# fernandezdaniel/MOBOCMF

Hardware: AMD Instinct MI355X
Metric: ELBO steps/sec (MFDGP d=8 M=512 N=8192 S=8) (higher is better)
Workload: dtype f64

## Files before the change

mobocmf_amd/csrc/common.h:

```cpp
#pragma once
#include <hip/hip_runtime.h>
#include <stdint.h>

#include "../../include/mobocmf_hip.h"

#define TILE 128
#define NB 64

static inline int64_t round_up(int64_t v, int64_t m) { return (v + m - 1) / m * m; }

#define HIP_TRY(expr)                                   \
    do {                                                \
        hipError_t _e = (expr);                         \
        if (_e != hipSuccess) return MOBOCMF_HIP_ERROR; \
    } while (0)

const mobocmf_tuning& tune();
bool tuning_ok(const mobocmf_tuning* t);
void probe_at(int i, hipStream_t s);
struct TuneScope {
    const mobocmf_tuning* prev_t;
    void* const* prev_p;
    explicit TuneScope(const mobocmf_tuning* t, void* const* probe = nullptr);
    ~TuneScope();
    TuneScope(const TuneScope&) = delete;
    TuneScope& operator=(const TuneScope&) = delete;
};

enum { TRI_NONE = 0, TRI_LOWER_A = 1, TRI_UPPER_A = 2, TRI_LOWER_B = 4, TRI_UPPER_B = 8 };
enum { EPI_STORE = 0, EPI_COLSTATS = 1, EPI_DA = 2 };

struct GemmArgs {
    const double* A;
    const double* B;
    double* C;
    int64_t lda, ldb, ldc;
    int Mr;
    int64_t Nc;
    int64_t Kd;
    int tri;
    int lower_out;
    int sym_out;
    int sym_full;
    int splitk_diag;
    double alpha;
    int accumulate;
    int rm;
    int pair_mode;
    int64_t slab_stride;
    int64_t strideA, strideB, strideC;
    int batched;
    int zlayers;
    int64_t zsA, zsB, zsC;
    const double* bscale;
    int64_t Kreal;
    double* rowdot_part;
    int stream_out;
    const int32_t* skip_if_zero;
    const int32_t* dual_flag;
    const double* bscale2;
    double* C2;
    const int32_t* colact;
    const int32_t* kact;
    int epi;
    double* colsq_part;
    double* coldot_part;
    const double* avec;
    const double* gmu;
    const double* cgv;
    const double* Aaux;
};

int launch_gemm(const GemmArgs& g, bool B_T, int splitk, hipStream_t s);
int gemm_nt_slabs(const GemmArgs& g, int splitk);
bool gemm_nt_is_small(const GemmArgs& g);
int gemm_rowdot_parts(const GemmArgs& g);
int gemm_colstat_rows(const GemmArgs& g);
int launch_gemm_auto(const GemmArgs& g, bool B_T, double* ws, int64_t ws_elems, hipStream_t s);
int launch_gemm_auto_pair(const GemmArgs& a, const GemmArgs& b, double* ws, int64_t ws_elems, hipStream_t s);

#define MAX_ZL 4

struct GramArgs {
    int kind, d, xdiv, zdiv;
    const double* x;
    const double* f;
    int64_t nbase;
    const double* Zx;
    const double* zf;
    int M;
    const double* hyp;
    double* K;
    int64_t ldk;
    int Mp;
    int64_t Np;
    double* knn;
    double jitter;
    int is_kmm;
    int gm;
    const double* G;
    const double* gknn;
    double* hyp_part;
    double* df_part;
    double* dzf_part;
    double* dx_part;
    const int32_t* colact;
};
int launch_gram_fwd(const GramArgs& g, hipStream_t s);
int launch_gram_bwd(const GramArgs& g, bool want_dx, hipStream_t s);
void gram_grid(const GramArgs& g, dim3* grid);
struct SumTask {
    const double* part; int64_t P, stride;
    const double* part2; int64_t P2, stride2;
    double* out; int64_t len; int accumulate;
    const double* extra;
};
int launch_sum_partials_multi(const SumTask* tasks, int n, hipStream_t s);

int launch_trtri(const double* L, int64_t ld, int Mp, const double* Dinv, double* Linv, double* T, double* ws,
                 int64_t ws_elems, hipStream_t s);
int launch_potrf_z(double* A, int64_t ld, int Mp, int M, double* Dinv, double* Ld, int32_t* const* info, int nz, int64_t zs,
                   double* zero0, double* zero1, void* sync, int* inverse_done, hipStream_t s);
int launch_trtri_z(const double* L, int64_t ld, int Mp, const double* Dinv, double* Linv, double* T, double* ws,
                   int64_t ws_elems, int nz, int64_t zs, hipStream_t s);

int launch_zero32(void* ptr, int64_t nwords, hipStream_t s);
int launch_pad_vec(const double* src, int64_t n, double* dst, int64_t np, hipStream_t s);
int launch_gemv_rows(const double* Mat, int64_t ld, const double* vec, double* out, int rows, int64_t cols, double scale,
                     int accumulate, hipStream_t s);
int launch_moments_finish(const double* qpart, const double* mupart, const double* rpart, int nrb, int64_t Np, int64_t N,
                          const double* knn, int branch, double min_var, double* q, double* r, double* varraw,
                          double* mean, double* var, int32_t* zero_word, hipStream_t s);
int launch_moments_bwd_prep(const double* g_mean, const double* g_var, const double* knn, const double* q,
                            const double* varraw, int branch, double min_var, int64_t N, int64_t Np, double* gmu,
                            double* gv, double* gv2, double* cgv, int32_t* nclamped, int zeroed, int32_t* blkact, hipStream_t s);
int launch_reduce_slabs_sym(const double* slabs, int64_t slab_stride, int nslab, int nslab_diag, double* out, int Mp, const int32_t* flag,
                            const double* fallback, hipStream_t s);
int launch_reduce_slabs_sym2(const double* slabs, const double* slabs2, int64_t slab_stride, int nslab, int nslab_diag,
                             double* out, double* out2, int Mp, const int32_t* flag, hipStream_t s);
int launch_copy_block(const double* src, int64_t lds, double* dst, int64_t ldd, int64_t rows, int64_t cols, hipStream_t s);
int launch_mf_combine(const double* Ks, const double* Kn, int64_t ld, const double* s1, const double* s2, const int32_t* l1,
                      const int32_t* l2, const double* ntab, int64_t n1, int64_t n2, double diag, double* out, int64_t ldo,
                      int64_t rows_p, int64_t cols_p, hipStream_t s);
int launch_copy_pad_identity(const double* src, int64_t lds, int n, double* dst, int np, hipStream_t s);
int launch_exact_gp_mll(const double* L, int64_t ld, const double* a, int n, double* mll, hipStream_t s);
int launch_exact_gp_finish(const double* qpart, const double* mupart, int nparts, int64_t ntp, int64_t nt, const double* kss,
                           double* mean, double* var, hipStream_t s);
int launch_mirror_lower(const double* src, int64_t lds, double* dst, int64_t ldd, int64_t row0, int64_t rows, int64_t cols,
                        int64_t n_real, hipStream_t s);
int launch_chain_outputs_z(const double* X, const double* LSp, const double* LinvT, const double* da_tot, int M, int Mp,
                           const double* const* gkl, double* const* gLS, double* const* gm, int nz, int64_t zs, hipStream_t s);
int launch_transpose_z(const double* in, int64_t ldi, double* out, int64_t ldo, int64_t rows, int64_t cols, int nz,
                       int64_t zs, hipStream_t s);
int launch_gemv_rows_z(const double* Mat, int64_t ld, const double* vec, double* out, int rows, int64_t cols, double scale,
                       int accumulate, int nz, int64_t zs, hipStream_t s);
int launch_transpose_pad_z(const double* in, double* out, int Mp, const double* const* LS, const double* const* m, int M,
                           double* LSp, double* mp, int nz, int64_t zs, hipStream_t s);
int launch_transpose_gemv_z(const double* in, double* out, int Mp, const double* Mat, const double* vec, double* vout, int nz,
                            int64_t zs, hipStream_t s);
int launch_kl_z(const double* L, const double* LSp, const double* U, const double* a, int M, int Mp, double* const* kl,
                double* part, int nz, int64_t zs, hipStream_t s);
int launch_dutot_y_z(const double* G1, const double* G2, const double* Hc, const double* U, const double* da, const double* a,
                     const double* const* gkl, int Mp, double* dU, double* da_tot, double* Y, int nz, int64_t zs, hipStream_t s);
int launch_dl_from_t2_z(const double* T2, const double* L, const double* const* gkl, int M, int Mp, double* dL, int nz,
                        int64_t zs, hipStream_t s);
int launch_phi_z(const double* T3, int Mp, double* P, int nz, int64_t zs, hipStream_t s);
int launch_symmetrize_z(const double* S, int Mp, double* G, int nz, int64_t zs, hipStream_t s);

enum { FCS_L = 0, FCS_LINV = 1, FCS_LINVT = 2, FCS_U = 3, FCS_UT = 4, FCS_LS = 5, FCS_A = 6 };
int launch_frozen_predict(const mobocmf_frozen_predict_model* host_models, const mobocmf_frozen_predict_model* dev_models,
                          int n_models, bool input_gradients, hipStream_t s);
int launch_frozen_predict_split(const mobocmf_frozen_predict_model* host_models, const mobocmf_frozen_predict_model* dev_models,
                                int n_models, bool input_gradients, hipStream_t s);

static inline int hyp_len(int kind, int d) { return kind == 0 ? 1 + d : 5 + 2 * d; }
#define MAX_D MOBOCMF_MAX_D

#define PHILOX_M0 0xD2511F53u
#define PHILOX_M1 0xCD9E8D57u
#define PHILOX_W0 0x9E3779B9u
#define PHILOX_W1 0xBB67AE85u
__device__ __forceinline__ void philox4x32_10(uint32_t c0, uint32_t c1, uint32_t c2, uint32_t c3, uint32_t k0, uint32_t k1,
                                              uint32_t (&out)[4]) {
#pragma unroll
    for (int r = 0; r < 10; ++r) {
        const uint32_t hi0 = __umulhi(PHILOX_M0, c0), lo0 = PHILOX_M0 * c0;
        const uint32_t hi1 = __umulhi(PHILOX_M1, c2), lo1 = PHILOX_M1 * c2;
        c0 = hi1 ^ c1 ^ k0; c1 = lo1; c2 = hi0 ^ c3 ^ k1; c3 = lo0;
        k0 += PHILOX_W0; k1 += PHILOX_W1;
    }
    out[0] = c0; out[1] = c1; out[2] = c2; out[3] = c3;
}
__device__ __forceinline__ double philox_normal(uint64_t seed, uint64_t call, uint64_t idx) {
    uint32_t r[4];
    philox4x32_10((uint32_t)idx, (uint32_t)(idx >> 32), (uint32_t)call, (uint32_t)(call >> 32), (uint32_t)seed,
                  (uint32_t)(seed >> 32), r);
    const double u1 = ((double)(((uint64_t)(r[0] >> 5) << 26) | (uint64_t)(r[1] >> 6)) + 0.5) * 1.1102230246251565e-16;
    const double u2 = ((double)(((uint64_t)(r[2] >> 5) << 26) | (uint64_t)(r[3] >> 6)) + 0.5) * 1.1102230246251565e-16;
    return sqrt(-2.0 * log(u1)) * cospi(2.0 * u2);
}
__device__ __forceinline__ double philox_uniform(uint64_t seed, uint64_t call, uint64_t idx) {
    uint32_t r[4];
    philox4x32_10((uint32_t)idx, (uint32_t)(idx >> 32), (uint32_t)call, (uint32_t)(call >> 32), (uint32_t)seed,
                  (uint32_t)(seed >> 32), r);
    return ((double)(((uint64_t)(r[0] >> 5) << 26) | (uint64_t)(r[1] >> 6)) + 0.5) * 1.1102230246251565e-16;
}
```

mobocmf_amd/csrc/gemm_f64.hip:

```cpp
#include "common.h"
#include <type_traits>
#include <atomic>

typedef double v4f64 __attribute__((ext_vector_type(4)));
typedef double v2f64 __attribute__((ext_vector_type(2)));

#define BM 128
#define BN 128
#define BK 16
#define KL_MAX 1024
#define TILE_ELEMS (BM * BK)

#define IMG_SWZ(row) ((((row) >> 1) & 1) | ((((row) >> 3) & 1) << 2))


template <int CTRL>
__device__ __forceinline__ double dpp_mov(double v) {
    int lo = __double2loint(v), hi = __double2hiint(v);
    lo = __builtin_amdgcn_update_dpp(0, lo, CTRL, 0xF, 0xF, false);
    hi = __builtin_amdgcn_update_dpp(0, hi, CTRL, 0xF, 0xF, false);
    return __hiloint2double(hi, lo);
}
__device__ __forceinline__ double row16_sum(double v) {
    v += dpp_mov<0xB1>(v);
    v += dpp_mov<0x4E>(v);
    v += dpp_mov<0x141>(v);
    v += dpp_mov<0x140>(v);
    return v;
}
__device__ __forceinline__ double rows4_sum(double v) {
    {
        const unsigned lo = (unsigned)__double2loint(v), hi = (unsigned)__double2hiint(v);
        const auto rl = __builtin_amdgcn_permlane16_swap(lo, lo, false, false);
        const auto rh = __builtin_amdgcn_permlane16_swap(hi, hi, false, false);
        v = __hiloint2double((int)rh[0], (int)rl[0]) + __hiloint2double((int)rh[1], (int)rl[1]);
    }
    {
        const unsigned lo = (unsigned)__double2loint(v), hi = (unsigned)__double2hiint(v);
        const auto rl = __builtin_amdgcn_permlane32_swap(lo, lo, false, false);
        const auto rh = __builtin_amdgcn_permlane32_swap(hi, hi, false, false);
        v = __hiloint2double((int)rh[0], (int)rl[0]) + __hiloint2double((int)rh[1], (int)rl[1]);
    }
    return v;
}

__device__ __forceinline__ void glds16(const double* gsrc, double* lds_wave_base) {
    __builtin_amdgcn_global_load_lds((const __attribute__((address_space(1))) void*)gsrc,
                                     (__attribute__((address_space(3))) void*)lds_wave_base, 16, 0, 0);
}

#ifdef GEMM_STAMPS
__device__ unsigned long long* g_stamp_buf = nullptr;
extern "C" int mobocmf_debug_set_stamps(unsigned long long* p) {
    return hipMemcpyToSymbol(HIP_SYMBOL(g_stamp_buf), &p, sizeof(p)) == hipSuccess ? 0 : 3;
}
#define STAMP(i)                                                                                            \
    do {                                                                                                    \
        if (g_stamp_buf && threadIdx.x == 0) g_stamp_buf[(int64_t)blockIdx.x * 32 + (i)] = __builtin_amdgcn_s_memrealtime(); \
    } while (0)
#define STAMP_ID()                                                                                          \
    do {                                                                                                    \
        if (g_stamp_buf && threadIdx.x == 0) {                                                              \
            unsigned hw, xcc;                                                                               \
            asm volatile("s_getreg_b32 %0, hwreg(HW_REG_HW_ID)" : "=s"(hw));                               \
            asm volatile("s_getreg_b32 %0, hwreg(HW_REG_XCC_ID)" : "=s"(xcc));                             \
            g_stamp_buf[(int64_t)blockIdx.x * 32 + 15] = ((unsigned long long)xcc << 32) | hw;              \
        }                                                                                                   \
    } while (0)
#define STEP_STAMPS_DECL unsigned long long sst[10] = {0, 0, 0, 0, 0, 0, 0, 0, 0, 0};
#define STEP_STAMP(i) do { if (sbase >= 0) sst[sbase + (i)] = __builtin_amdgcn_s_memrealtime(); } while (0)
#define STEP_STAMPS_FLUSH                                                                                   \
    do {                                                                                                    \
        if (g_stamp_buf && threadIdx.x == 0)                                                                \
            for (int q = 0; q < 10; ++q) g_stamp_buf[(int64_t)blockIdx.x * 32 + 16 + q] = sst[q];           \
    } while (0)
#else
#define STAMP(i)
#define STAMP_ID()
#define STEP_STAMPS_DECL
#define STEP_STAMP(i)
#define STEP_STAMPS_FLUSH
#endif

template <bool B_T, bool TRI, int EPI, int RM>
__global__ __launch_bounds__(256, RM == 64 ? 3 : 2) void gemm_f64_kernel(GemmArgs g, int nrb, int64_t ncb, int splitk, int pair) {
    static_assert(RM == 128 || (RM == 64 && !B_T), "tile heights: 128, or 64 for the A B form");
    constexpr int MT = RM / 32;
    constexpr int A_ELEMS = RM * BK;
    constexpr int STAGE_ELEMS = A_ELEMS + TILE_ELEMS;
    __shared__ __attribute__((aligned(16))) double lds[2 * STAGE_ELEMS];
    __shared__ int kl[B_T ? KL_MAX : 1];
    __shared__ int kl_wsum[4];
    if (g.skip_if_zero && *g.skip_if_zero == 0) return;
    STAMP(0);
    STAMP_ID();
    int64_t id = blockIdx.x;
    if (g.dual_flag) {
        const int64_t half = (int64_t)(gridDim.x >> 1);
        if (id >= half) {
            if (*g.dual_flag == 0) return;
            id -= half;
            g.bscale = g.bscale2;
            g.C = g.C2;
        }
    }
    int rb, z = 0, sk_eff = splitk;
    int64_t cb;
    if (g.batched) {
        z = blockIdx.z;
        cb = id / nrb;
        rb = nrb - 1 - (int)(id % nrb);
    } else if (splitk > 1 && g.lower_out && g.splitk_diag > 0) {
        const int64_t nF = (int64_t)nrb * (nrb - 1) / 2, nblkF = nF * splitk;
        const bool diag = id >= nblkF;
        const int64_t id2 = diag ? id - nblkF : id, nT = diag ? nrb : nF;
        sk_eff = diag ? g.splitk_diag : splitk;
        int64_t t;
        if ((sk_eff & 7) == 0 && (nblkF & 7) == 0) {
            const int64_t xcd = id2 & 7, seq = id2 >> 3;
            t = seq % nT;
            z = (int)((seq / nT) * 8 + xcd);
        } else {
            t = id2 % nT;
            z = (int)(id2 / nT);
        }
        if (diag) {
            rb = (int)t;
            cb = t;
        } else {
            int r = 1;
            while ((int64_t)r * (r + 1) / 2 <= t) ++r;
            rb = r;
            cb = t - (int64_t)r * (r - 1) / 2;
        }
    } else if (splitk > 1) {
        const int64_t ntile = g.lower_out ? (int64_t)nrb * (nrb + 1) / 2 : (int64_t)nrb * ncb;
        int64_t t;
        if ((splitk & 7) == 0) {
            const int64_t xcd = id & 7, seq = id >> 3;
            t = seq % ntile;
            z = (int)((seq / ntile) * 8 + xcd);
        } else {
            t = id % ntile;
            z = (int)(id / ntile);
        }
        if (g.lower_out) {
            int r = 0;
            while ((int64_t)(r + 1) * (r + 2) / 2 <= t) ++r;
            rb = r;
            cb = t - (int64_t)r * (r + 1) / 2;
        } else {
            cb = t / nrb;
            rb = (int)(t % nrb);
        }
    } else {
        const int nslot = pair ? (nrb + 1) / 2 : nrb;
        int sl;
        if ((ncb & 7) == 0) {
            int64_t xcd = id & 7, slot = id >> 3;
            cb = (slot / nslot) * 8 + xcd;
            sl = (int)(slot % nslot);
        } else {
            cb = id / nslot;
            sl = (int)(id % nslot);
        }
        rb = pair ? sl : nrb - 1 - sl;
    }
    if (g.lower_out && cb > rb) return;

    const double* A = g.A;
    const double* B = g.B;
    double* C = g.C;
    if (g.batched) {
        const int zl = g.zlayers > 1 ? z % g.zlayers : 0;
        const int zb = g.zlayers > 1 ? z / g.zlayers : z;
        A += zb * g.strideA + zl * g.zsA;
        B += zb * g.strideB + zl * g.zsB;
        C += zb * g.strideC + zl * g.zsC;
    }
    if (!g.batched && splitk > 1) {
        C += z * g.slab_stride;
        if (g.zlayers > 1) {
            A += blockIdx.z * g.zsA;
            B += blockIdx.z * g.zsB;
            C += blockIdx.z * g.zsC;
        }
    }
    const int nparts = (pair && rb != nrb - 1 - rb) ? 2 : 1;
    const int rb_first = rb;

    const int tid = threadIdx.x;
    const int lane = tid & 63;
    const int wave = __builtin_amdgcn_readfirstlane(tid >> 6);
    const int wr = wave >> 1, wc = wave & 1;
    const int li = lane & 15, lk = lane >> 4;

    if constexpr (!B_T) {
        if (g.colact && g.colact[cb] == 0) {
            if (EPI == EPI_DA && g.rowdot_part) {
                for (int part = 0; part < nparts; ++part) {
                    const int rbp = part == 0 ? rb_first : nrb - 1 - rb_first;
                    for (int i = tid; i < 2 * RM; i += 256)
                        g.rowdot_part[((int64_t)cb * 2 + i / RM) * g.Mr + (int64_t)rbp * RM + i % RM] = 0.0;
                }
            }
            return;
        }
    }

    const int a_row = tid >> 3;
    const int a_lchk = (tid & 7) ^ IMG_SWZ(a_row);
    const double* Ag0 = A + (int64_t)a_row * g.lda + a_lchk * 2;
    const double* Bg = B_T ? B + (cb * BN + a_row) * g.ldb + a_lchk * 2
                           : B + (int64_t)wave * g.ldb + cb * BN;
    auto stage = [&](const double* Ag, int64_t k, int buf) {
        double* As = lds + buf * STAGE_ELEMS;
        double* Bs = As + A_ELEMS;
#pragma unroll
        for (int r = 0; r < RM / 32; ++r) glds16(Ag + (int64_t)(32 * r) * g.lda + k, As + (r * 4 + wave) * 128);
        if (B_T) {
#pragma unroll
            for (int r = 0; r < 4; ++r) glds16(Bg + (int64_t)(32 * r) * g.ldb + k, Bs + (r * 4 + wave) * 128);
        } else {
#pragma unroll
            for (int r = 0; r < 4; ++r)
                glds16(Bg + (k + 4 * r) * g.ldb + lane * 2, Bs + (r * 4 + wave) * 128);
        }
    };

    const int swA = IMG_SWZ(li);
    const int colP0 = ((2 * lk + 0) ^ swA) << 1, colP1 = ((2 * lk + 1) ^ swA) << 1;
    const int a_base = (wr * 16 + li) * BK;
    const int bt_base = (wc * 16 + li) * BK;
    const int bn_base = (4 * lk) * BN + wc * 64 + 2 * li;

  STEP_STAMPS_DECL
  for (int part = 0; part < nparts; ++part) {
    const bool upper = (g.tri & TRI_UPPER_A) != 0;
    const bool long_first_is_high = !upper;
    rb = ((part == 0) == long_first_is_high) ? nrb - 1 - rb_first : rb_first;
    if (nparts == 1) rb = rb_first;
    const bool rev = TRI && nparts == 2 && (upper ? part == 0 : part == 1);
    int64_t k0 = 0, k1 = g.Kd;
    if (g.tri & TRI_LOWER_A) {
        int64_t e = (int64_t)(rb + 1) * RM;
        if (k1 > e) k1 = e;
    }
    if (g.tri & TRI_UPPER_A) {
        int64_t b = (int64_t)rb * RM;
        if (k0 < b) k0 = b;
    }
    if (g.tri & TRI_LOWER_B) {
        int64_t b = cb * BN;
        if (k0 < b) k0 = b;
    }
    if (g.tri & TRI_UPPER_B) {
        int64_t e = (cb + 1) * BN;
        if (k1 > e) k1 = e;
    }
    bool compact = false;
    int64_t ct0 = 0;
    int co0 = 0;
    if (!g.batched && splitk > 1) {
        bool sliced = false;
        if constexpr (B_T) {
            if (g.kact) {
                const int nb = (int)(g.Kd / 128), run = (nb + 255) / 256;
                const int rb0 = tid * run < nb ? tid * run : nb, rb1 = rb0 + run < nb ? rb0 + run : nb;
                int cnt = 0;
                for (int b = rb0; b < rb1; ++b) cnt += g.kact[b] != 0 ? 1 : 0;
                int inc = cnt;
#pragma unroll
                for (int off = 1; off < 64; off <<= 1) {
                    const int v = __shfl_up(inc, off);
                    if (lane >= off) inc += v;
                }
                if (lane == 63) kl_wsum[wave] = inc;
                __syncthreads();
                int ord = inc - cnt;
                for (int w = 0; w < wave; ++w) ord += kl_wsum[w];
                const int64_t nkt = (int64_t)(kl_wsum[0] + kl_wsum[1] + kl_wsum[2] + kl_wsum[3]) * (128 / BK);
                const int64_t per = (nkt + sk_eff - 1) / sk_eff;
                const int64_t tb = z * per < nkt ? z * per : nkt, te = tb + per < nkt ? tb + per : nkt;
                ct0 = tb;
                co0 = (int)(tb / (128 / BK));
                const int co1 = te > tb ? (int)((te - 1) / (128 / BK)) : co0 - 1;
                for (int b = rb0; b < rb1; ++b)
                    if (g.kact[b] != 0) {
                        if (ord >= co0 && ord <= co1 && ord - co0 < KL_MAX) kl[ord - co0] = b;
                        ++ord;
                    }
                __syncthreads();
                compact = true;
                sliced = true;
                k0 = 0;
                k1 = (te - tb) * BK;
            }
        }
        if (!sliced) {
            int64_t nkt = k1 > k0 ? (k1 - k0) / BK : 0;
            int64_t per = (nkt + sk_eff - 1) / sk_eff;
            int64_t b = k0 + z * per * BK, e = b + per * BK;
            k0 = b < k1 ? b : k1;
            k1 = e < k1 ? e : k1;
        }
    }
    const double* Ag = Ag0 + (int64_t)rb * RM * g.lda;

    v4f64 acc[MT][4];
#pragma unroll
    for (int i = 0; i < MT; ++i)
#pragma unroll
        for (int j = 0; j < 4; ++j) acc[i][j] = (v4f64){0.0, 0.0, 0.0, 0.0};

    const int64_t nk = (k1 > k0) ? (k1 - k0) / BK : 0;
#define KSTEP(KT) (rev ? nk - 1 - (KT) : (KT))
    auto koff = [&](int64_t kt) -> int64_t {
        if (B_T && compact) {
            const int64_t t = ct0 + kt;
            return (int64_t)kl[(int)(t / (128 / BK)) - co0] * 128 + (t % (128 / BK)) * BK;
        }
        return k0 + KSTEP(kt) * BK;
    };
#define KOFF(KT) koff(KT)
    if (nk > 0) stage(Ag, KOFF(0), 0);

    asm volatile("s_waitcnt vmcnt(0)" ::: "memory");
    __syncthreads();
    STAMP(1 + 4 * part);
    v4f64 w_nxt = (v4f64){1.0, 1.0, 1.0, 1.0};
    if (B_T && g.bscale && nk > 0) w_nxt = *(const v4f64*)(g.bscale + KOFF(0) + 4 * lk);
    v2f64 fa[MT][2];
    double fb[4][4];
#define LOAD_A16(MT_)                                                                                       \
    fa[MT_][0] = *(const v2f64*)(As + a_base + (MT_) * 32 * BK + colP0);                                    \
    fa[MT_][1] = *(const v2f64*)(As + a_base + (MT_) * 32 * BK + colP1);
#define LOAD_B16                                                                                            \
    if (B_T) {                                                                                              \
        _Pragma("unroll") for (int t = 0; t < 4; ++t) {                                                    \
            const v2f64 v0 = *(const v2f64*)(Bs + bt_base + t * 32 * BK + colP0);                           \
            const v2f64 v1 = *(const v2f64*)(Bs + bt_base + t * 32 * BK + colP1);                           \
            fb[0][t] = v0[0];                                                                               \
            fb[1][t] = v0[1];                                                                               \
            fb[2][t] = v1[0];                                                                               \
            fb[3][t] = v1[1];                                                                               \
        }                                                                                                   \
        if (g.bscale) {                                                                                     \
// ... 1073 lines not shown
```

mobocmf_amd/csrc/gram.hip:

```cpp
#include "common.h"

#define GT 128
#define GM 32


typedef double v2f64_t __attribute__((ext_vector_type(2)));

template <int KIND, int DB, int XD>
__global__ __launch_bounds__(GT) void gram_fwd_kernel(GramArgs g) {
    __shared__ __attribute__((aligned(16))) double stg[XD ? (GT / 64) * 64 * (XD + 2) : 1];
    __shared__ double zs[GM][DB];
    __shared__ double zfs[GM];
    __shared__ double il1[DB], il2[DB];
    const int d = g.d;
    const int tid = threadIdx.x;
    const int gm = g.gm;
    const int m0 = blockIdx.y * gm;
    const double* hyp = g.hyp;
    double a1, af = 0, nu = 0, a2 = 0, ilf = 0;
    if (KIND == 0) {
        a1 = hyp[0];
        if (tid < DB) il1[tid] = tid < d ? 1.0 / hyp[1 + tid] : 0.0;
    } else {
        a1 = hyp[0]; af = hyp[1]; nu = hyp[2]; a2 = hyp[3]; ilf = 1.0 / hyp[4];
        if (tid < DB) { il1[tid] = tid < d ? 1.0 / hyp[5 + tid] : 0.0; il2[tid] = tid < d ? 1.0 / hyp[5 + d + tid] : 0.0; }
    }
    for (int e = tid; e < gm * DB; e += GT) {
        int mm = e / DB, k = e % DB;
        int m = m0 + mm;
        zs[mm][k] = (m < g.M && k < d) ? g.Zx[(int64_t)(m / g.zdiv) * d + k] : 0.0;
    }
    if (KIND == 1 && tid < gm) zfs[tid] = (m0 + tid < g.M) ? g.zf[m0 + tid] : 0.0;
    __syncthreads();

    const int64_t n0 = (int64_t)blockIdx.x * GT + tid;
    const int xdiv = XD ? XD : g.xdiv;
    const int64_t c0 = n0 * xdiv;
    if (c0 >= g.Np) return;
    const bool real = n0 < g.nbase;
    double xr[DB];
#pragma unroll
    for (int k = 0; k < DB; ++k) xr[k] = (real && k < d) ? g.x[n0 * d + k] : 0.0;
    double fr[XD ? XD : 1];
    if (XD && KIND == 1) {
#pragma unroll
        for (int s = 0; s < XD; s += 2) {
            v2f64_t v = real ? *(const v2f64_t*)(g.f + c0 + s) : (v2f64_t){0.0, 0.0};
            fr[s] = v[0];
            fr[s + 1] = v[1];
        }
    }

    const bool full_wave = XD && __ballot(real) == ~0ull;
    (void)full_wave;
    if (g.knn && blockIdx.y == 0) {
        for (int s = 0; s < xdiv; ++s) {
            int64_t n = c0 + s;
            if (n >= g.Np) break;
            double v = 0.0;
            if (real) {
                if (KIND == 0) v = a1;
                else { double fn = g.f[n]; v = a1 * (nu * fn * fn + af) + a2; }
            }
            g.knn[n] = v;
        }
    }
    for (int mm = 0; mm < gm; ++mm) {
        const int m = m0 + mm;
        double* krow = g.K + (int64_t)m * g.ldk;
        if (!real || m >= g.M) {
            for (int s = 0; s < xdiv; ++s) {
                int64_t n = c0 + s;
                if (n >= g.Np) break;
                krow[n] = (g.is_kmm && n == m) ? 1.0 : 0.0;
            }
            continue;
        }
        double d1 = 0.0, d2 = 0.0;
#pragma unroll
        for (int k = 0; k < DB; ++k) {
            double df = xr[k] - zs[mm][k];
            double t1 = df * il1[k];
            d1 += t1 * t1;
            if (KIND == 1) { double t2 = df * il2[k]; d2 += t2 * t2; }
        }
        const double E1 = exp(-0.5 * d1);
        if (KIND == 0) {
            double v = a1 * E1;
            if (g.is_kmm && c0 == m) v += g.jitter;
            krow[c0] = v;
            for (int s = 1; s < xdiv; ++s) krow[c0 + s] = a1 * E1;
        } else if (XD) {
            const double E2 = exp(-0.5 * d2);
            const double zfm = zfs[mm];
            const double c1 = a1 * E1, c2 = a2 * E2;
            const double cp = c1 * nu * zfm, cq = c1 * af;
            const int lane = tid & 63;
            double* my = stg + (tid >> 6) * 64 * (XD + 2);
#pragma unroll
            for (int s = 0; s < XD; s += 2) {
                v2f64_t v;
#pragma unroll
                for (int e = 0; e < 2; ++e) {
                    const double fn = fr[s + e];
                    const double fd = (fn - zfm) * ilf;
                    v[e] = cq * exp(-0.5 * fd * fd) + (cp * fn + c2);
                }
                if (full_wave) *(v2f64_t*)(my + lane * (XD + 2) + s) = v;
                else *(v2f64_t*)(krow + c0 + s) = v;
            }
            if (full_wave) {
                double* wrow = krow + (c0 - (int64_t)lane * XD);
#pragma unroll
                for (int i = 0; i < XD / 2; ++i) {
                    const int e = (i * 64 + lane) * 2;
                    *(v2f64_t*)(wrow + e) = *(const v2f64_t*)(my + (e / XD) * (XD + 2) + e % XD);
                }
            }
        } else {
            const double E2 = exp(-0.5 * d2);
            const double zfm = zfs[mm];
            const double c1 = a1 * E1, c2 = a2 * E2;
            for (int s = 0; s < xdiv; ++s) {
                const int64_t n = c0 + s;
                const double fn = g.f[n];
                const double fd = (fn - zfm) * ilf;
                const double Ef = exp(-0.5 * fd * fd);
                double v = c1 * (nu * fn * zfm + af * Ef) + c2;
                if (g.is_kmm && n == m) v += g.jitter;
                krow[n] = v;
            }
        }
    }
}

__device__ __forceinline__ double wave_sum(double v) {
    v += __shfl_xor(v, 1);
    v += __shfl_xor(v, 2);
    v += __shfl_xor(v, 4);
    v += __shfl_xor(v, 8);
    v += __shfl_xor(v, 16);
    v += __shfl_xor(v, 32);
    return v;
}

template <int KIND, int DB, bool WANT_DX, int XD>
__global__ __launch_bounds__(GT) void gram_bwd_kernel(GramArgs g) {
    __shared__ double zs[GM][DB];
    __shared__ double zfs[GM];
    __shared__ double il1[DB], il2[DB];
    __shared__ double dzf_s[GM];
    __shared__ double red[2][8 + 2 * DB];
    extern __shared__ double dfs[];
    const int d = g.d;
    const int tid = threadIdx.x, lane = tid & 63, wave = tid >> 6;
    const int gm = g.gm;
    const int m0 = blockIdx.y * gm;
    const double* hyp = g.hyp;
    double a1, af = 0, nu = 0, a2 = 0, ilf = 0;
    if (KIND == 0) {
        a1 = hyp[0];
        if (tid < DB) il1[tid] = tid < d ? 1.0 / hyp[1 + tid] : 0.0;
    } else {
        a1 = hyp[0]; af = hyp[1]; nu = hyp[2]; a2 = hyp[3]; ilf = 1.0 / hyp[4];
        if (tid < DB) { il1[tid] = tid < d ? 1.0 / hyp[5 + tid] : 0.0; il2[tid] = tid < d ? 1.0 / hyp[5 + d + tid] : 0.0; }
    }
    for (int e = tid; e < gm * DB; e += GT) {
        int mm = e / DB, k = e % DB;
        int m = m0 + mm;
        zs[mm][k] = (m < g.M && k < d) ? g.Zx[(int64_t)(m / g.zdiv) * d + k] : 0.0;
    }
    if (tid < gm) {
        dzf_s[tid] = 0.0;
        if (KIND == 1) zfs[tid] = (m0 + tid < g.M) ? g.zf[m0 + tid] : 0.0;
    }
    __syncthreads();

    const int64_t n0 = (int64_t)blockIdx.x * GT + tid;
    const int xdiv = XD ? XD : g.xdiv;
    const int64_t c0 = n0 * xdiv;
    const bool real = n0 < g.nbase;
    static_assert(XD == 0 || 128 % XD == 0, "replica runs must not straddle a column block");
    unsigned long long amask = ~0ull;
    if (g.colact && real) {
        if (XD) amask = g.colact[c0 >> 7] != 0 ? ~0ull : 0ull;
        else {
            amask = 0ull;
            for (int s = 0; s < xdiv; ++s) amask |= (unsigned long long)(g.colact[(c0 + s) >> 7] != 0 ? 1 : 0) << s;
        }
    }
    const bool live = real && amask != 0ull;
    double fr[XD ? XD : 1], dfa[XD ? XD : 1];
    if (XD) {
#pragma unroll
        for (int s = 0; s < XD; s += 2) {
            v2f64_t v = real ? *(const v2f64_t*)(g.f + c0 + s) : (v2f64_t){0.0, 0.0};
            fr[s] = v[0];
            fr[s + 1] = v[1];
            dfa[s] = dfa[s + 1] = 0.0;
        }
    }
    double xr[DB], aL1[DB], aL2[KIND == 1 ? DB : 1], aX[WANT_DX ? DB : 1];
#pragma unroll
    for (int k = 0; k < DB; ++k) {
        xr[k] = (real && k < d) ? g.x[n0 * d + k] : 0.0;
        aL1[k] = 0.0;
        if (KIND == 1) aL2[k] = 0.0;
        if (WANT_DX) aX[k] = 0.0;
    }
    double s_a1 = 0, s_af = 0, s_nu = 0, s_a2 = 0, s_lsf = 0;
    if (KIND == 1 && !XD)
        for (int s = 0; s < xdiv; ++s) dfs[s * GT + tid] = 0.0;

    if (g.gknn && blockIdx.y == 0 && real) {
        for (int s = 0; s < xdiv; ++s) {
            const int64_t n = c0 + s;
            const double gk = g.gknn[n];
            if (KIND == 0) s_a1 += gk;
            else {
                const double fn = g.f[n];
                s_a1 += gk * (nu * fn * fn + af);
                s_nu += gk * a1 * fn * fn;
                s_af += gk * a1;
                s_a2 += gk;
            }
        }
    }

    for (int mm = 0; mm < gm; ++mm) {
        const int m = m0 + mm;
        if (m >= g.M) break;
        double dzf_loc = 0.0;
        if (live) {
            const double* grow = g.G + (int64_t)m * g.ldk;
            double d1 = 0.0, d2 = 0.0;
#pragma unroll
            for (int k = 0; k < DB; ++k) {
                double df = xr[k] - zs[mm][k];
                double t1 = df * il1[k];
                d1 += t1 * t1;
                if (KIND == 1) { double t2 = df * il2[k]; d2 += t2 * t2; }
            }
            const double E1 = exp(-0.5 * d1);
            double W1 = 0.0, W2 = 0.0;
            if (KIND == 0) {
                double Gsum = 0.0;
                for (int s = 0; s < xdiv; ++s) Gsum += ((amask >> s) & 1ull) ? grow[c0 + s] : 0.0;
                s_a1 += Gsum * E1;
                W1 = Gsum * a1 * E1;
            } else {
                const double E2 = exp(-0.5 * d2);
                const double zfm = zfs[mm];
                const double aE1 = a1 * E1;
                const double c_a = aE1 * nu * zfm, c_b = aE1 * af * ilf;
                double G2s = 0.0, S1 = 0.0, S2 = 0.0, S3 = 0.0, S4 = 0.0;
                auto body = [&](double Gv, double fn, double& dfacc) {
                    const double fd = (fn - zfm) * ilf;
                    const double GEf = Gv * exp(-0.5 * fd * fd);
                    const double T = GEf * fd;
                    G2s += Gv;
                    S1 += Gv * fn;
                    S2 += GEf;
                    S3 += T;
                    S4 += T * fd;
                    dfacc += Gv * c_a - T * c_b;
                };
                if (XD) {
#pragma unroll
                    for (int s = 0; s < XD; s += 2) {
                        const v2f64_t Gp = *(const v2f64_t*)(grow + c0 + s);
                        body(Gp[0], fr[s], dfa[s]);
                        body(Gp[1], fr[s + 1], dfa[s + 1]);
                    }
                } else {
                    for (int s = 0; s < xdiv; ++s) {
                        double acc = 0.0;
                        body(((amask >> s) & 1ull) ? grow[c0 + s] : 0.0, g.f[c0 + s], acc);
                        dfs[s * GT + tid] += acc;
                    }
                }
                const double inner = nu * zfm * S1 + af * S2;
                s_a1 += E1 * inner;
                s_nu += aE1 * zfm * S1;
                s_af += aE1 * S2;
                s_lsf += c_b * S4;
                W1 = aE1 * inner;
                dzf_loc = aE1 * nu * S1 + c_b * S3;
                s_a2 += G2s * E2;
                W2 = G2s * a2 * E2;
            }
#pragma unroll
            for (int k = 0; k < DB; ++k) {
                double df = xr[k] - zs[mm][k];
                double t1 = df * il1[k];
                aL1[k] += W1 * t1 * t1;
                double gx = W1 * t1 * il1[k];
                if (KIND == 1) {
                    double t2 = df * il2[k];
                    aL2[k] += W2 * t2 * t2;
                    gx += W2 * t2 * il2[k];
                }
                if (WANT_DX) aX[k] -= gx;
            }
        }
        if (KIND == 1) {
            double tot = wave_sum(dzf_loc);
            if (lane == 0) atomicAdd(&dzf_s[mm], tot);
        }
    }
    if (KIND == 1) {
        for (int s = 0; s < xdiv; ++s) {
            const int64_t n = c0 + s;
            if (n >= g.Np) break;
            double v = real ? (XD ? dfa[XD ? s : 0] : dfs[s * GT + tid]) : 0.0;
            if (real && g.gknn && blockIdx.y == 0) v += g.gknn[n] * a1 * 2.0 * nu * g.f[n];
            g.df_part[(int64_t)blockIdx.y * g.Np + n] = v;
        }
    }
    if (WANT_DX && real) {
        double* dxp = g.dx_part + ((int64_t)blockIdx.y * g.nbase + n0) * d;
#pragma unroll
        for (int k = 0; k < DB; ++k)
            if (k < d) dxp[k] = aX[k];
    }
    const int H = (KIND == 0) ? 1 + d : 5 + 2 * d;
    {
        double v;
        v = wave_sum(s_a1); if (lane == 0) red[wave][0] = v;
        if (KIND == 1) {
            v = wave_sum(s_af); if (lane == 0) red[wave][1] = v;
            v = wave_sum(s_nu); if (lane == 0) red[wave][2] = v;
            v = wave_sum(s_a2); if (lane == 0) red[wave][3] = v;
            v = wave_sum(s_lsf); if (lane == 0) red[wave][4] = v;
        }
#pragma unroll
        for (int k = 0; k < DB; ++k) {
            if (k < d) {
                v = wave_sum(aL1[k]);
                if (lane == 0) red[wave][(KIND == 0 ? 1 : 5) + k] = v * il1[k];
                if (KIND == 1) {
                    v = wave_sum(aL2[k]);
                    if (lane == 0) red[wave][5 + d + k] = v * il2[k];
                }
            }
        }
    }
    __syncthreads();
    double* hp = g.hyp_part + ((int64_t)blockIdx.y * gridDim.x + blockIdx.x) * H;
    if (tid < H) hp[tid] = red[0][tid] + red[1][tid];
    if (KIND == 1 && tid < gm) g.dzf_part[(int64_t)blockIdx.x * g.Mp + m0 + tid] = dzf_s[tid];
}

#define SUM_MULTI_MAX 8
struct SumTasksArg { SumTask t[SUM_MULTI_MAX]; int blk0[SUM_MULTI_MAX + 1]; int wide[SUM_MULTI_MAX]; int n; };
__global__ void sum_partials_multi_kernel(SumTasksArg T) {
    __shared__ double sh[4];
    int k = 0;
    while (k + 1 < T.n && (int)blockIdx.x >= T.blk0[k + 1]) ++k;
    const SumTask& t = T.t[k];
    if (T.wide[k] == 1) {
        const int64_t j = (int64_t)(blockIdx.x - T.blk0[k]);
        double v = 0.0;
        for (int64_t p = threadIdx.x; p < t.P; p += 256) v += t.part[p * t.stride + j];
        if (t.part2)
            for (int64_t p = threadIdx.x; p < t.P2; p += 256) v += t.part2[p * t.stride2 + j];
        v += __shfl_xor(v, 1); v += __shfl_xor(v, 2); v += __shfl_xor(v, 4);
        v += __shfl_xor(v, 8); v += __shfl_xor(v, 16); v += __shfl_xor(v, 32);
        if ((threadIdx.x & 63) == 0) sh[threadIdx.x >> 6] = v;
        __syncthreads();
        if (threadIdx.x == 0) {
            v = sh[0] + sh[1] + sh[2] + sh[3];
            if (t.extra) v += t.extra[j];
            t.out[j] = t.accumulate ? t.out[j] + v : v;
        }
        return;
    }
    if (T.wide[k] == 2) {
        __shared__ double sq[4][64];
        const int jj = threadIdx.x & 63, q = threadIdx.x >> 6;
        const int64_t j = (int64_t)(blockIdx.x - T.blk0[k]) * 64 + jj;
        double v = 0.0;
        if (j < t.len) {
            for (int64_t p = q; p < t.P; p += 4) v += t.part[p * t.stride + j];
            if (t.part2)
                for (int64_t p = q; p < t.P2; p += 4) v += t.part2[p * t.stride2 + j];
        }
        sq[q][jj] = v;
        __syncthreads();
        if (q == 0 && j < t.len) {
            v = (sq[0][jj] + sq[1][jj]) + (sq[2][jj] + sq[3][jj]);
            if (t.extra) v += t.extra[j];
            t.out[j] = t.accumulate ? t.out[j] + v : v;
        }
        return;
    }
    const int64_t j = (int64_t)(blockIdx.x - T.blk0[k]) * blockDim.x + threadIdx.x;
    if (j >= t.len) return;
    double v = 0.0;
    for (int64_t p = 0; p < t.P; ++p) v += t.part[p * t.stride + j];
    if (t.part2)
        for (int64_t p = 0; p < t.P2; ++p) v += t.part2[p * t.stride2 + j];
    if (t.extra) v += t.extra[j];
    t.out[j] = t.accumulate ? t.out[j] + v : v;
}

int launch_sum_partials_multi(const SumTask* tasks, int n, hipStream_t s) {
    if (n > SUM_MULTI_MAX) {
        for (int i = 0; i < n; i += SUM_MULTI_MAX) {
            int rc = launch_sum_partials_multi(tasks + i, n - i < SUM_MULTI_MAX ? n - i : SUM_MULTI_MAX, s);
            if (rc) return rc;
        }
        return MOBOCMF_OK;
    }
    SumTasksArg T = {};
    int64_t nb = 0;
    int m = 0;
    for (int i = 0; i < n; ++i) {
        if (tasks[i].len <= 0) continue;
        T.t[m] = tasks[i];
        T.blk0[m] = (int)nb;
        const int64_t pmax = tasks[i].P > (tasks[i].part2 ? tasks[i].P2 : 0) ? tasks[i].P : tasks[i].P2;
        T.wide[m] = (pmax >= 64 && tasks[i].len <= 4096) ? 1 : (pmax >= 16 ? 2 : 0);
        nb += T.wide[m] == 1 ? tasks[i].len : T.wide[m] == 2 ? (tasks[i].len + 63) / 64 : (tasks[i].len + 255) / 256;
        ++m;
    }
    T.blk0[m] = (int)nb;
    T.n = m;
    if (m == 0) return MOBOCMF_OK;
    if (nb > 0x7fffffff) return MOBOCMF_BAD_ARG;
    hipLaunchKernelGGL(sum_partials_multi_kernel, dim3((unsigned)nb), dim3(256), 0, s, T);
    return hipGetLastError() == hipSuccess ? MOBOCMF_OK : MOBOCMF_HIP_ERROR;
}

static inline int d_bucket(int d) { return d <= 2 ? 2 : (d <= 8 ? 8 : 32); }

static int gram_rows_per_block(const GramArgs& g, bool fwd = false) {
    int64_t nb_cols = (g.Np + g.xdiv - 1) / g.xdiv;
    int64_t gx = (nb_cols + GT - 1) / GT;
    int gm = GM;
    while (gm > GM / 4 && gx * (g.Mp / gm) < 1024) gm /= 2;
    if (fwd && g.is_kmm)
        while (gm > 2 && gx * (g.Mp / gm) < 4096) gm /= 2;
    return gm;
}
void gram_grid(const GramArgs& g, dim3* grid) {
    int64_t nb_cols = (g.Np + g.xdiv - 1) / g.xdiv;
    *grid = dim3((unsigned)((nb_cols + GT - 1) / GT), (unsigned)(g.Mp / gram_rows_per_block(g)), 1);
}

int launch_gram_fwd(const GramArgs& g0, hipStream_t s) {
    GramArgs g = g0;
    g.gm = gram_rows_per_block(g0, true);
    if (g.d < 1 || g.d > 32) return MOBOCMF_BAD_ARG;
    dim3 grid;
    gram_grid(g, &grid);
    grid.y = (unsigned)(g.Mp / g.gm);
    const int db = d_bucket(g.d);
#define GF(K, D, X) hipLaunchKernelGGL((gram_fwd_kernel<K, D, X>), grid, dim3(GT), 0, s, g)
    const bool vec_ok = g.kind == 1 && !g.is_kmm && ((uintptr_t)g.f % 16 == 0) && ((uintptr_t)g.K % 16 == 0) && (g.ldk % 2 == 0);
    if (g.kind == 0) { if (db == 2) GF(0, 2, 0); else if (db == 8) GF(0, 8, 0); else GF(0, 32, 0); }
    else if (vec_ok && g.xdiv == 8) { if (db == 2) GF(1, 2, 8); else if (db == 8) GF(1, 8, 8); else GF(1, 32, 8); }
    else if (vec_ok && g.xdiv == 16) { if (db == 2) GF(1, 2, 16); else if (db == 8) GF(1, 8, 16); else GF(1, 32, 16); }
    else { if (db == 2) GF(1, 2, 0); else if (db == 8) GF(1, 8, 0); else GF(1, 32, 0); }
#undef GF
    return hipGetLastError() == hipSuccess ? MOBOCMF_OK : MOBOCMF_HIP_ERROR;
}

int launch_gram_bwd(const GramArgs& g0, bool want_dx, hipStream_t s) {
    GramArgs g = g0;
    g.gm = gram_rows_per_block(g0);
    if (g.d < 1 || g.d > 32) return MOBOCMF_BAD_ARG;
    dim3 grid;
    gram_grid(g, &grid);
    const int db = d_bucket(g.d);
    if (g.xdiv > 48) return MOBOCMF_BAD_ARG;
    const size_t shm = g.kind == 1 ? (size_t)g.xdiv * GT * sizeof(double) : 0;
#define GB(K, D, X)                                                                                    \
    do {                                                                                               \
        if (want_dx) hipLaunchKernelGGL((gram_bwd_kernel<K, D, true, X>), grid, dim3(GT), (X) ? 0 : shm, s, g);   \
        else hipLaunchKernelGGL((gram_bwd_kernel<K, D, false, X>), grid, dim3(GT), (X) ? 0 : shm, s, g);          \
    } while (0)
    const bool vec_ok = g.kind == 1 && ((uintptr_t)g.f % 16 == 0) && ((uintptr_t)g.G % 16 == 0) && (g.ldk % 2 == 0);
    if (g.kind == 0) { if (db == 2) GB(0, 2, 0); else if (db == 8) GB(0, 8, 0); else GB(0, 32, 0); }
    else if (vec_ok && g.xdiv == 8) { if (db == 2) GB(1, 2, 8); else if (db == 8) GB(1, 8, 8); else GB(1, 32, 8); }
    else if (vec_ok && g.xdiv == 16) { if (db == 2) GB(1, 2, 16); else if (db == 8) GB(1, 8, 16); else GB(1, 32, 16); }
    else { if (db == 2) GB(1, 2, 0); else if (db == 8) GB(1, 8, 0); else GB(1, 32, 0); }
#undef GB
    return hipGetLastError() == hipSuccess ? MOBOCMF_OK : MOBOCMF_HIP_ERROR;
}
```

Baseline: 1070.

## Restructure gram backward: stage G rows in LDS, prefetch, DPP reductions

Reworks the Gram backward kernel. It adds an XD==1 specialization that stages the block's G rows into shared memory up front. For XD>1 it software-prefetches the next G row into registers and keeps df accumulators in LDS instead of registers, and it vectorizes the x loads. Wave reductions now use DPP and permlane swaps instead of shfl_xor, and occupancy hints are added to launch_bounds. This targets load latency and register pressure in the backward pass, at the cost of more LDS use and template variants.

```diff
diff --git a/mobocmf_amd/csrc/common.h b/mobocmf_amd/csrc/common.h
--- a/mobocmf_amd/csrc/common.h
+++ b/mobocmf_amd/csrc/common.h
@@ -26,6 +26,37 @@
     TuneScope(const TuneScope&) = delete;
     TuneScope& operator=(const TuneScope&) = delete;
 };
+
+template <int CTRL>
+__device__ __forceinline__ double dpp_mov(double v) {
+    int lo = __double2loint(v), hi = __double2hiint(v);
+    lo = __builtin_amdgcn_update_dpp(0, lo, CTRL, 0xF, 0xF, false);
+    hi = __builtin_amdgcn_update_dpp(0, hi, CTRL, 0xF, 0xF, false);
+    return __hiloint2double(hi, lo);
+}
+__device__ __forceinline__ double row16_sum(double v) {
+    v += dpp_mov<0xB1>(v);
+    v += dpp_mov<0x4E>(v);
+    v += dpp_mov<0x141>(v);
+    v += dpp_mov<0x140>(v);
+    return v;
+}
+__device__ __forceinline__ double rows4_sum(double v) {
+    {
+        const unsigned lo = (unsigned)__double2loint(v), hi = (unsigned)__double2hiint(v);
+        const auto rl = __builtin_amdgcn_permlane16_swap(lo, lo, false, false);
+        const auto rh = __builtin_amdgcn_permlane16_swap(hi, hi, false, false);
+        v = __hiloint2double((int)rh[0], (int)rl[0]) + __hiloint2double((int)rh[1], (int)rl[1]);
+    }
+    {
+        const unsigned lo = (unsigned)__double2loint(v), hi = (unsigned)__double2hiint(v);
+        const auto rl = __builtin_amdgcn_permlane32_swap(lo, lo, false, false);
+        const auto rh = __builtin_amdgcn_permlane32_swap(hi, hi, false, false);
+        v = __hiloint2double((int)rh[0], (int)rl[0]) + __hiloint2double((int)rh[1], (int)rl[1]);
+    }
+    return v;
+}
+__device__ __forceinline__ double wave_sum_dpp(double v) { return rows4_sum(row16_sum(v)); }
 
 enum { TRI_NONE = 0, TRI_LOWER_A = 1, TRI_UPPER_A = 2, TRI_LOWER_B = 4, TRI_UPPER_B = 8 };
 enum { EPI_STORE = 0, EPI_COLSTATS = 1, EPI_DA = 2 };
@@ -98,6 +129,7 @@
     double jitter;
     int is_kmm;
     int gm;
+    int xvec;
     const double* G;
     const double* gknn;
     double* hyp_part;
diff --git a/mobocmf_amd/csrc/gemm_f64.hip b/mobocmf_amd/csrc/gemm_f64.hip
--- a/mobocmf_amd/csrc/gemm_f64.hip
+++ b/mobocmf_amd/csrc/gemm_f64.hip
@@ -13,36 +13,6 @@
 
 #define IMG_SWZ(row) ((((row) >> 1) & 1) | ((((row) >> 3) & 1) << 2))
 
-
-template <int CTRL>
-__device__ __forceinline__ double dpp_mov(double v) {
-    int lo = __double2loint(v), hi = __double2hiint(v);
-    lo = __builtin_amdgcn_update_dpp(0, lo, CTRL, 0xF, 0xF, false);
-    hi = __builtin_amdgcn_update_dpp(0, hi, CTRL, 0xF, 0xF, false);
-    return __hiloint2double(hi, lo);
-}
-__device__ __forceinline__ double row16_sum(double v) {
-    v += dpp_mov<0xB1>(v);
-    v += dpp_mov<0x4E>(v);
-    v += dpp_mov<0x141>(v);
-    v += dpp_mov<0x140>(v);
-    return v;
-}
-__device__ __forceinline__ double rows4_sum(double v) {
-    {
-        const unsigned lo = (unsigned)__double2loint(v), hi = (unsigned)__double2hiint(v);
-        const auto rl = __builtin_amdgcn_permlane16_swap(lo, lo, false, false);
-        const auto rh = __builtin_amdgcn_permlane16_swap(hi, hi, false, false);
-        v = __hiloint2double((int)rh[0], (int)rl[0]) + __hiloint2double((int)rh[1], (int)rl[1]);
-    }
-    {
-        const unsigned lo = (unsigned)__double2loint(v), hi = (unsigned)__double2hiint(v);
-        const auto rl = __builtin_amdgcn_permlane32_swap(lo, lo, false, false);
-        const auto rh = __builtin_amdgcn_permlane32_swap(hi, hi, false, false);
-        v = __hiloint2double((int)rh[0], (int)rl[0]) + __hiloint2double((int)rh[1], (int)rl[1]);
-    }
-    return v;
-}
 
 __device__ __forceinline__ void glds16(const double* gsrc, double* lds_wave_base) {
     __builtin_amdgcn_global_load_lds((const __attribute__((address_space(1))) void*)gsrc,
diff --git a/mobocmf_amd/csrc/gram.hip b/mobocmf_amd/csrc/gram.hip
--- a/mobocmf_amd/csrc/gram.hip
+++ b/mobocmf_amd/csrc/gram.hip
@@ -134,18 +134,9 @@
     }
 }
 
-__device__ __forceinline__ double wave_sum(double v) {
-    v += __shfl_xor(v, 1);
-    v += __shfl_xor(v, 2);
-    v += __shfl_xor(v, 4);
-    v += __shfl_xor(v, 8);
-    v += __shfl_xor(v, 16);
-    v += __shfl_xor(v, 32);
-    return v;
-}
-
 template <int KIND, int DB, bool WANT_DX, int XD>
-__global__ __launch_bounds__(GT) void gram_bwd_kernel(GramArgs g) {
+__global__ __launch_bounds__(GT, (XD > 1 && DB <= 8 ? (XD * DB <= 64 ? 3 : 2) : 1)) void gram_bwd_kernel(GramArgs g) {
+    constexpr int XS = XD == 1 ? 1 : 2;
     __shared__ double zs[GM][DB];
     __shared__ double zfs[GM];
     __shared__ double il1[DB], il2[DB];
@@ -190,26 +181,48 @@
         }
     }
     const bool live = real && amask != 0ull;
-    double fr[XD ? XD : 1], dfa[XD ? XD : 1];
-    if (XD) {
-#pragma unroll
-        for (int s = 0; s < XD; s += 2) {
-            v2f64_t v = real ? *(const v2f64_t*)(g.f + c0 + s) : (v2f64_t){0.0, 0.0};
-            fr[s] = v[0];
-            fr[s + 1] = v[1];
-            dfa[s] = dfa[s + 1] = 0.0;
+    const int64_t nr = real ? n0 : 0;
+    double fr[XD ? XD : 1], dfa = 0.0;
+    if (XD && KIND == 1) {
+        const double* fp = g.f + nr * XD;
+#pragma unroll
+        for (int s = 0; s < XD; s += XS) {
+            if (XS == 1) fr[s] = real ? fp[s] : 0.0;
+            else {
+                const v2f64_t v = *(const v2f64_t*)(fp + s);
+                fr[s] = real ? v[0] : 0.0;
+                fr[s + XS - 1] = real ? v[1] : 0.0;
+            }
         }
     }
     double xr[DB], aL1[DB], aL2[KIND == 1 ? DB : 1], aX[WANT_DX ? DB : 1];
+    {
+        const double* xp = g.x + nr * d;
+        if (g.xvec) {
+#pragma unroll
+            for (int k = 0; k < DB; k += 2) {
+                v2f64_t v = {0.0, 0.0};
+                if (k < d) v = *(const v2f64_t*)(xp + k);
+                xr[k] = real ? v[0] : 0.0;
+                xr[k + 1] = real ? v[1] : 0.0;
+            }
+        } else {
+#pragma unroll
+            for (int k = 0; k < DB; ++k) {
+                double v = 0.0;
+                if (k < d) v = xp[k];
+                xr[k] = real ? v : 0.0;
+            }
+        }
+    }
 #pragma unroll
     for (int k = 0; k < DB; ++k) {
-        xr[k] = (real && k < d) ? g.x[n0 * d + k] : 0.0;
         aL1[k] = 0.0;
         if (KIND == 1) aL2[k] = 0.0;
         if (WANT_DX) aX[k] = 0.0;
     }
     double s_a1 = 0, s_af = 0, s_nu = 0, s_a2 = 0, s_lsf = 0;
-    if (KIND == 1 && !XD)
+    if (KIND == 1 && XD != 1)
         for (int s = 0; s < xdiv; ++s) dfs[s * GT + tid] = 0.0;
 
     if (g.gknn && blockIdx.y == 0 && real) {
@@ -227,12 +240,38 @@
         }
     }
 
-    for (int mm = 0; mm < gm; ++mm) {
-        const int m = m0 + mm;
-        if (m >= g.M) break;
+    const int rows = min(gm, g.M - m0);
+    const double* gcol = g.G + (int64_t)m0 * g.ldk + c0;
+    double Gq[XD > 1 ? XD : 1];
+    auto g_fetch = [&](int s, int row) {
+        const v2f64_t v = *(const v2f64_t*)(gcol + (int64_t)(row < gm ? row : gm - 1) * g.ldk + s);
+        Gq[s] = v[0];
+        Gq[s + XS - 1] = v[1];
+    };
+    if (XD == 1 && live) {
+        auto stage = [&](int r0, auto R) {
+            double t[R.value];
+#pragma unroll
+            for (int e = 0; e < R.value; ++e) t[e] = gcol[(int64_t)(r0 + e) * g.ldk];
+#pragma unroll
+            for (int e = 0; e < R.value; ++e) dfs[(r0 + e) * GT + tid] = t[e];
+        };
+        if (gm == 32) stage(0, std::integral_constant<int, 32>{});
+        else if (gm == 16) stage(0, std::integral_constant<int, 16>{});
+        else {
+            int r0 = 0;
+            for (; r0 + 8 <= gm; r0 += 8) stage(r0, std::integral_constant<int, 8>{});
+            for (; r0 < gm; ++r0) stage(r0, std::integral_constant<int, 1>{});
+        }
+    }
+    if (XD > 1 && live) {
+#pragma unroll
+        for (int s = 0; s < XD; s += XS) g_fetch(s, 0);
+    }
+    for (int mm = 0; mm < rows; ++mm) {
         double dzf_loc = 0.0;
         if (live) {
-            const double* grow = g.G + (int64_t)m * g.ldk;
+            const double* grow = gcol + (int64_t)mm * g.ldk - c0;
             double d1 = 0.0, d2 = 0.0;
 #pragma unroll
             for (int k = 0; k < DB; ++k) {
@@ -245,7 +284,30 @@
             double W1 = 0.0, W2 = 0.0;
             if (KIND == 0) {
                 double Gsum = 0.0;
-                for (int s = 0; s < xdiv; ++s) Gsum += ((amask >> s) & 1ull) ? grow[c0 + s] : 0.0;
+                if (XD) {
+#pragma unroll
+                    for (int s = 0; s < XD; s += XS) {
+                        if (XD == 1) Gsum += dfs[mm * GT + tid];
+                        else {
+                            Gsum += Gq[s];
+                            Gsum += Gq[s + XS - 1];
+                            g_fetch(s, mm + 1);
+                        }
+                    }
+                } else {
+                    for (int s0 = 0; s0 < xdiv; s0 += 4) {
+                        double Gc[4];
+#pragma unroll
+                        for (int e = 0; e < 4; ++e) {
+                            const int sc = s0 + e < xdiv ? s0 + e : xdiv - 1;
+                            const double v = grow[c0 + sc];
+                            Gc[e] = ((amask >> sc) & 1ull) ? v : 0.0;
+                        }
+#pragma unroll
+                        for (int e = 0; e < 4; ++e)
+                            if (s0 + e < xdiv) Gsum += Gc[e];
+                    }
+                }
                 s_a1 += Gsum * E1;
                 W1 = Gsum * a1 * E1;
             } else {
@@ -265,18 +327,39 @@
                     S4 += T * fd;
                     dfacc += Gv * c_a - T * c_b;
                 };
-                if (XD) {
+                if (XD == 1) {
+                    double acc = 0.0;
+                    body(dfs[mm * GT + tid], fr[0], acc);
+                    dfa += acc;
+                } else if (XD) {
 #pragma unroll
                     for (int s = 0; s < XD; s += 2) {
-                        const v2f64_t Gp = *(const v2f64_t*)(grow + c0 + s);
-                        body(Gp[0], fr[s], dfa[s]);
-                        body(Gp[1], fr[s + 1], dfa[s + 1]);
+                        double acc0 = dfs[s * GT + tid], acc1 = dfs[(s + XS - 1) * GT + tid];
+                        body(Gq[s], fr[s], acc0);
+                        body(Gq[s + XS - 1], fr[s + XS - 1], acc1);
+                        dfs[s * GT + tid] = acc0;
+                        dfs[(s + XS - 1) * GT + tid] = acc1;
+                        g_fetch(s, mm + 1);
+                        __builtin_amdgcn_sched_barrier(0);
                     }
                 } else {
-                    for (int s = 0; s < xdiv; ++s) {
-                        double acc = 0.0;
-                        body(((amask >> s) & 1ull) ? grow[c0 + s] : 0.0, g.f[c0 + s], acc);
-                        dfs[s * GT + tid] += acc;
+                    for (int s0 = 0; s0 < xdiv; s0 += 4) {
+                        double Gc[4], fc[4];
+#pragma unroll
+                        for (int e = 0; e < 4; ++e) {
+                            const int sc = s0 + e < xdiv ? s0 + e : xdiv - 1;
+                            const double v = grow[c0 + sc];
+                            Gc[e] = ((amask >> sc) & 1ull) ? v : 0.0;
+                            fc[e] = g.f[c0 + sc];
+                        }
+#pragma unroll
+                        for (int e = 0; e < 4; ++e) {
+                            if (s0 + e < xdiv) {
+                                double acc = 0.0;
+                                body(Gc[e], fc[e], acc);
+                                dfs[(s0 + e) * GT + tid] += acc;
+                            }
+                        }
                     }
                 }
                 const double inner = nu * zfm * S1 + af * S2;
@@ -289,6 +372,10 @@
                 s_a2 += G2s * E2;
                 W2 = G2s * a2 * E2;
             }
+            if (KIND == 1) {
+#pragma unroll
+                for (int k = 0; k < DB; ++k) asm volatile("" : "+v"(xr[k]));
+            }
 #pragma unroll
             for (int k = 0; k < DB; ++k) {
                 double df = xr[k] - zs[mm][k];
@@ -304,7 +391,7 @@
             }
         }
         if (KIND == 1) {
-            double tot = wave_sum(dzf_loc);
+            double tot = wave_sum_dpp(dzf_loc);
             if (lane == 0) atomicAdd(&dzf_s[mm], tot);
         }
     }
@@ -312,7 +399,7 @@
         for (int s = 0; s < xdiv; ++s) {
             const int64_t n = c0 + s;
             if (n >= g.Np) break;
-            double v = real ? (XD ? dfa[XD ? s : 0] : dfs[s * GT + tid]) : 0.0;
+            double v = real ? (XD == 1 ? dfa : dfs[s * GT + tid]) : 0.0;
             if (real && g.gknn && blockIdx.y == 0) v += g.gknn[n] * a1 * 2.0 * nu * g.f[n];
             g.df_part[(int64_t)blockIdx.y * g.Np + n] = v;
         }
@@ -326,20 +413,20 @@
     const int H = (KIND == 0) ? 1 + d : 5 + 2 * d;
     {
         double v;
-        v = wave_sum(s_a1); if (lane == 0) red[wave][0] = v;
+        v = wave_sum_dpp(s_a1); if (lane == 0) red[wave][0] = v;
         if (KIND == 1) {
-            v = wave_sum(s_af); if (lane == 0) red[wave][1] = v;
-            v = wave_sum(s_nu); if (lane == 0) red[wave][2] = v;
-            v = wave_sum(s_a2); if (lane == 0) red[wave][3] = v;
-            v = wave_sum(s_lsf); if (lane == 0) red[wave][4] = v;
+            v = wave_sum_dpp(s_af); if (lane == 0) red[wave][1] = v;
+            v = wave_sum_dpp(s_nu); if (lane == 0) red[wave][2] = v;
+            v = wave_sum_dpp(s_a2); if (lane == 0) red[wave][3] = v;
+            v = wave_sum_dpp(s_lsf); if (lane == 0) red[wave][4] = v;
         }
 #pragma unroll
         for (int k = 0; k < DB; ++k) {
             if (k < d) {
-                v = wave_sum(aL1[k]);
+                v = wave_sum_dpp(aL1[k]);
                 if (lane == 0) red[wave][(KIND == 0 ? 1 : 5) + k] = v * il1[k];
                 if (KIND == 1) {
-                    v = wave_sum(aL2[k]);
+                    v = wave_sum_dpp(aL2[k]);
                     if (lane == 0) red[wave][5 + d + k] = v * il2[k];
                 }
             }
@@ -474,14 +561,17 @@
     gram_grid(g, &grid);
     const int db = d_bucket(g.d);
     if (g.xdiv > 48) return MOBOCMF_BAD_ARG;
-    const size_t shm = g.kind == 1 ? (size_t)g.xdiv * GT * sizeof(double) : 0;
+    const size_t shm = (g.xdiv == 1 ? (size_t)g.gm : g.kind == 1 ? (size_t)g.xdiv : 0) * GT * sizeof(double);
 #define GB(K, D, X)                                                                                    \
     do {                                                                                               \
-        if (want_dx) hipLaunchKernelGGL((gram_bwd_kernel<K, D, true, X>), grid, dim3(GT), (X) ? 0 : shm, s, g);   \
-        else hipLaunchKernelGGL((gram_bwd_kernel<K, D, false, X>), grid, dim3(GT), (X) ? 0 : shm, s, g);          \
+        if (want_dx) hipLaunchKernelGGL((gram_bwd_kernel<K, D, true, X>), grid, dim3(GT), shm, s, g);   \
+        else hipLaunchKernelGGL((gram_bwd_kernel<K, D, false, X>), grid, dim3(GT), shm, s, g);          \
     } while (0)
     const bool vec_ok = g.kind == 1 && ((uintptr_t)g.f % 16 == 0) && ((uintptr_t)g.G % 16 == 0) && (g.ldk % 2 == 0);
-    if (g.kind == 0) { if (db == 2) GB(0, 2, 0); else if (db == 8) GB(0, 8, 0); else GB(0, 32, 0); }
+    g.xvec = ((uintptr_t)g.x % 16 == 0) && (g.d % 2 == 0);
+    if (g.kind == 0 && g.xdiv == 1) { if (db == 2) GB(0, 2, 1); else if (db == 8) GB(0, 8, 1); else GB(0, 32, 1); }
+    else if (g.kind == 0) { if (db == 2) GB(0, 2, 0); else if (db == 8) GB(0, 8, 0); else GB(0, 32, 0); }
+    else if (g.xdiv == 1) { if (db == 2) GB(1, 2, 1); else if (db == 8) GB(1, 8, 1); else GB(1, 32, 1); }
     else if (vec_ok && g.xdiv == 8) { if (db == 2) GB(1, 2, 8); else if (db == 8) GB(1, 8, 8); else GB(1, 32, 8); }
     else if (vec_ok && g.xdiv == 16) { if (db == 2) GB(1, 2, 16); else if (db == 8) GB(1, 8, 16); else GB(1, 32, 16); }
     else { if (db == 2) GB(1, 2, 0); else if (db == 8) GB(1, 8, 0); else GB(1, 32, 0); }
```

New measurement: 1074 (median of 6 runs). About the same (+0.4%).
